# WHU-USI3DV/LaneMapping

Hardware: AMD Instinct MI355X
Metric: BEV tiles/sec end-to-end (LAS points -> polylines) (higher is better)
Workload: dtype f32; 1 GPU; on-GPU LAS->BEV raster (4,194,304 points/tile resident in HBM) + configs/Proj_polyline_fpn_vit_vertex_2.py, batch=16 per GPU, seeded random weights; lines_per_tile=45, streams=2, hip_graphs=True, points=resident, stream_check=not run (--full runs it), gather_check=n/a (1 rank), raster_check=not run (--full runs it), dist_ranks=1, rccl_ranks=1

## Files before the change

### lanemapping_amd/csrc/vit.hip

```cpp
#include "common.h"

namespace {

constexpr int DH = 64;
constexpr int QC = 36;
constexpr int KLD = DH + 1;
constexpr size_t VALU_STATIC_LDS = 272;
constexpr size_t LDS_PER_WG = 160 * 1024;
constexpr size_t valu_dynamic_lds(int N) { return ((size_t)N * KLD + (size_t)QC * (N + 4) + QC * DH) * sizeof(float); }
constexpr bool valu_fits(int N) { return valu_dynamic_lds(N) + VALU_STATIC_LDS <= LDS_PER_WG; }
static_assert(valu_fits(380) && !valu_fits(381), "the VALU kernel holds 380 keys (163312 + 272 B), not 381 (163716 + 272 B > 163840)");
static_assert(valu_fits(64), "the masked entry's 64 tokens fit");

__global__ __launch_bounds__(256) void attention_kernel(const float* __restrict__ qkv, float* __restrict__ out, int NT,
                                                        int heads, float scale, const int* __restrict__ valid) {
    extern __shared__ __attribute__((aligned(16))) float smem[];
    __shared__ int kidx[64];
    __shared__ int kcount;
    const int tid = threadIdx.x;
    const int q0 = blockIdx.x * QC, h = blockIdx.y, b = blockIdx.z;
    const int inner = heads * DH;
    const long row0 = (long)b * NT;
    const int ld = 3 * inner;
    int N = NT;
    if (valid) {
        if (tid < 64) {
            const bool v = tid < NT && valid[(long)b * NT + tid] != 0;
            const unsigned long long m = __ballot(v);
            if (v) kidx[__popcll(m & ((1ull << tid) - 1ull))] = tid;
            if (tid == 0) kcount = (int)__popcll(m);
        }
        __syncthreads();
        N = kcount;
        if (N == 0) {
            for (int i = tid; i < QC * DH; i += 256) {
                const int n = q0 + (i >> 6);
                if (n < NT) out[(row0 + n) * inner + h * DH + (i & 63)] = 0.f;
            }
            return;
        }
    }
    const int SLD = N + 4;
    float* KV = smem;
    float* S = KV + N * KLD;
    float* Q = S + QC * SLD;
#define LM_KROW(n) (valid ? kidx[n] : (n))

    for (int i = tid; i < N * DH; i += 256) {
        const int n = i >> 6, d = i & 63;
        KV[n * KLD + d] = qkv[(row0 + LM_KROW(n)) * ld + inner + h * DH + d];
    }
    for (int i = tid; i < QC * DH; i += 256) {
        const int n = i >> 6, d = i & 63;
        Q[i] = (q0 + n < NT) ? qkv[(row0 + q0 + n) * ld + h * DH + d] : 0.f;
    }
    __syncthreads();
    for (int idx = tid; idx < QC * N; idx += 256) {
        const int i = idx / N, j = idx - i * N;
        const float* qr = Q + i * DH;
        const float* kr = KV + j * KLD;
        float acc = 0.f;
#pragma unroll
        for (int d = 0; d < DH; ++d) acc = fmaf(qr[d], kr[d], acc);
        S[i * SLD + j] = acc * scale;
    }
    __syncthreads();
    for (int i = tid; i < N * DH; i += 256) {
        const int n = i >> 6, d = i & 63;
        KV[n * KLD + d] = qkv[(row0 + LM_KROW(n)) * ld + 2 * inner + h * DH + d];
    }
#undef LM_KROW
    const int wave = tid >> 6, lane = tid & 63;
    for (int i = wave; i < QC; i += 4) {
        float* sr = S + i * SLD;
        float m = -INFINITY;
        for (int j = lane; j < N; j += 64) m = fmaxf(m, sr[j]);
        for (int o = 32; o > 0; o >>= 1) m = fmaxf(m, __shfl_xor(m, o));
        float sum = 0.f;
        for (int j = lane; j < N; j += 64) {
            const float e = expf(sr[j] - m);
            sr[j] = e;
            sum += e;
        }
        for (int o = 32; o > 0; o >>= 1) sum += __shfl_xor(sum, o);
        const float inv = 1.0f / sum;
        for (int j = lane; j < N; j += 64) sr[j] *= inv;
    }
    __syncthreads();
    const int d = lane;
    float acc[QC / 4];
#pragma unroll
    for (int r = 0; r < QC / 4; ++r) acc[r] = 0.f;
    for (int j = 0; j < N; ++j) {
        const float v = KV[j * KLD + d];
#pragma unroll
        for (int r = 0; r < QC / 4; ++r) acc[r] = fmaf(S[(wave + 4 * r) * SLD + j], v, acc[r]);
    }
#pragma unroll
    for (int r = 0; r < QC / 4; ++r) {
        const int i = q0 + wave + 4 * r;
        if (i < NT) out[(row0 + i) * inner + h * DH + d] = acc[r];
    }
}

typedef float f32x16 __attribute__((ext_vector_type(16)));
typedef float f32x4 __attribute__((ext_vector_type(4)));
constexpr int NKB = 11;
constexpr int NPAD = NKB * 32;
constexpr int KP = DH + 4;

__global__ __launch_bounds__(256) void attention_mfma_kernel(const float* __restrict__ qkv, float* __restrict__ out, int N, int heads,
                                                             float scale) {
    extern __shared__ __attribute__((aligned(16))) float smem[];
    const int tid = threadIdx.x, lane = tid & 63, wave = tid >> 6;
    const int h = blockIdx.y, b = blockIdx.z;
    const int inner = heads * DH, ld = 3 * inner;
    const long row0 = (long)b * N;
    const int col = lane & 31, half = lane >> 5;
    const int q = (blockIdx.x * 4 + wave) * 32 + col;
    for (int i = tid; i < NPAD * (DH / 4); i += 256) {
        const int n = i >> 4, c4 = (i & 15) * 4;
        f32x4 v = {0.f, 0.f, 0.f, 0.f};
        if (n < N) v = *reinterpret_cast<const f32x4*>(qkv + (row0 + n) * ld + inner + h * DH + c4);
        *reinterpret_cast<f32x4*>(smem + n * KP + c4) = v;
    }
    f32x4 qf[8];
#pragma unroll
    for (int g = 0; g < 8; ++g) {
        qf[g] = f32x4{0.f, 0.f, 0.f, 0.f};
        if (q < N) qf[g] = *reinterpret_cast<const f32x4*>(qkv + (row0 + q) * ld + h * DH + 8 * g + 4 * half);
    }
    __syncthreads();
    f32x16 s[NKB];
#pragma unroll
    for (int kb = 0; kb < NKB; ++kb) {
#pragma unroll
        for (int r = 0; r < 16; ++r) s[kb][r] = 0.f;
#pragma unroll
        for (int g = 0; g < 8; ++g) {
            const f32x4 kf = *reinterpret_cast<const f32x4*>(smem + (kb * 32 + col) * KP + 8 * g + 4 * half);
#pragma unroll
            for (int t = 0; t < 4; ++t) s[kb] = __builtin_amdgcn_mfma_f32_32x32x2f32(kf[t], qf[g][t], s[kb], 0, 0, 0);
        }
    }
    float m = -INFINITY;
#pragma unroll
    for (int kb = 0; kb < NKB; ++kb)
#pragma unroll
        for (int r = 0; r < 16; ++r) {
            const int key = kb * 32 + (r & 3) + 8 * (r >> 2) + 4 * half;
            s[kb][r] = key < N ? s[kb][r] * scale : -INFINITY;
            m = fmaxf(m, s[kb][r]);
        }
    m = fmaxf(m, __shfl_xor(m, 32));
    float sum = 0.f;
#pragma unroll
    for (int kb = 0; kb < NKB; ++kb)
#pragma unroll
        for (int r = 0; r < 16; ++r) {
            const float e = expf(s[kb][r] - m);
            s[kb][r] = e;
            sum += e;
        }
    sum += __shfl_xor(sum, 32);
    __syncthreads();
    for (int i = tid; i < NPAD * (DH / 4); i += 256) {
        const int n = i >> 4, c4 = (i & 15) * 4;
        f32x4 v = {0.f, 0.f, 0.f, 0.f};
        if (n < N) v = *reinterpret_cast<const f32x4*>(qkv + (row0 + n) * ld + 2 * inner + h * DH + c4);
        *reinterpret_cast<f32x4*>(smem + n * DH + c4) = v;
    }
    __syncthreads();
    f32x16 o[2];
#pragma unroll
    for (int dt = 0; dt < 2; ++dt)
#pragma unroll
        for (int r = 0; r < 16; ++r) o[dt][r] = 0.f;
#pragma unroll
    for (int kb = 0; kb < NKB; ++kb)
#pragma unroll
        for (int r = 0; r < 16; ++r) {
            const float* vrow = smem + (kb * 32 + (r & 3) + 8 * (r >> 2) + 4 * half) * DH + col;
            o[0] = __builtin_amdgcn_mfma_f32_32x32x2f32(vrow[0], s[kb][r], o[0], 0, 0, 0);
            o[1] = __builtin_amdgcn_mfma_f32_32x32x2f32(vrow[32], s[kb][r], o[1], 0, 0, 0);
        }
    if (q < N) {
        const float inv = 1.0f / sum;
        float* orow = out + (row0 + q) * inner + h * DH;
#pragma unroll
        for (int dt = 0; dt < 2; ++dt)
#pragma unroll
            for (int r4 = 0; r4 < 4; ++r4) {
                f32x4 v = {o[dt][4 * r4] * inv, o[dt][4 * r4 + 1] * inv, o[dt][4 * r4 + 2] * inv, o[dt][4 * r4 + 3] * inv};
                *reinterpret_cast<f32x4*>(orow + dt * 32 + 8 * r4 + 4 * half) = v;
            }
    }
}

constexpr int FKB = 64;
constexpr int VP = DH + 8;

__global__ __launch_bounds__(256) __attribute__((amdgpu_waves_per_eu(4))) void attention_flash_kernel(
    const float* __restrict__ qkv, float* __restrict__ out, int N, int heads, float scale) {
    extern __shared__ __attribute__((aligned(16))) float smem[];
    float* Ks = smem;
    float* Vs = smem + FKB * KP;
    const int tid = threadIdx.x, lane = tid & 63, wave = tid >> 6;
    const int h = blockIdx.y, b = blockIdx.z;
    const int inner = heads * DH, ld = 3 * inner;
    const long row0 = (long)b * N;
    const int col = lane & 31, half = lane >> 5;
    const int q = (blockIdx.x * 4 + wave) * 32 + col;
    f32x4 qf[8];
#pragma unroll
    for (int g = 0; g < 8; ++g) {
        qf[g] = f32x4{0.f, 0.f, 0.f, 0.f};
        if (q < N) qf[g] = *reinterpret_cast<const f32x4*>(qkv + (row0 + q) * ld + h * DH + 8 * g + 4 * half);
    }
    f32x16 o[2];
#pragma unroll
    for (int dt = 0; dt < 2; ++dt)
#pragma unroll
        for (int r = 0; r < 16; ++r) o[dt][r] = 0.f;
    float m = -INFINITY, l = 0.f;
    for (int k0 = 0; k0 < N; k0 += FKB) {
        __syncthreads();
        for (int i = tid; i < FKB * (DH / 4); i += 256) {
            const int n = i >> 4, c4 = (i & 15) * 4;
            f32x4 kv = {0.f, 0.f, 0.f, 0.f}, vv = {0.f, 0.f, 0.f, 0.f};
            if (k0 + n < N) {
                const float* src = qkv + (row0 + k0 + n) * ld + inner + h * DH + c4;
                kv = *reinterpret_cast<const f32x4*>(src);
                vv = *reinterpret_cast<const f32x4*>(src + inner);
            }
            *reinterpret_cast<f32x4*>(Ks + n * KP + c4) = kv;
            *reinterpret_cast<f32x4*>(Vs + n * VP + c4) = vv;
        }
        __syncthreads();
#pragma unroll
        for (int sb = 0; sb < FKB / 32; ++sb) {
            const int kb0 = k0 + sb * 32;
            if (kb0 >= N) break;
            f32x16 s;
#pragma unroll
            for (int r = 0; r < 16; ++r) s[r] = 0.f;
#pragma unroll
            for (int g = 0; g < 8; ++g) {
                const f32x4 kf = *reinterpret_cast<const f32x4*>(Ks + (sb * 32 + col) * KP + 8 * g + 4 * half);
#pragma unroll
                for (int t = 0; t < 4; ++t) s = __builtin_amdgcn_mfma_f32_32x32x2f32(kf[t], qf[g][t], s, 0, 0, 0);
            }
            float mb = m;
#pragma unroll
            for (int r = 0; r < 16; ++r) {
                const int key = kb0 + (r & 3) + 8 * (r >> 2) + 4 * half;
                s[r] = key < N ? s[r] * scale : -INFINITY;
                mb = fmaxf(mb, s[r]);
            }
            mb = fmaxf(mb, __shfl_xor(mb, 32));
            const float alpha = expf(m - mb);
            m = mb;
            float ps = 0.f;
#pragma unroll
            for (int r = 0; r < 16; ++r) {
                s[r] = expf(s[r] - m);
                ps += s[r];
            }
            l = l * alpha + ps;
            o[0] *= alpha;
            o[1] *= alpha;
#pragma unroll
            for (int r = 0; r < 16; ++r) {
                const float* vrow = Vs + (sb * 32 + (r & 3) + 8 * (r >> 2) + 4 * half) * VP + col;
                o[0] = __builtin_amdgcn_mfma_f32_32x32x2f32(vrow[0], s[r], o[0], 0, 0, 0);
                o[1] = __builtin_amdgcn_mfma_f32_32x32x2f32(vrow[32], s[r], o[1], 0, 0, 0);
            }
        }
    }
    l += __shfl_xor(l, 32);
    if (q < N) {
        const float inv = 1.0f / l;
        float* orow = out + (row0 + q) * inner + h * DH;
#pragma unroll
        for (int dt = 0; dt < 2; ++dt)
#pragma unroll
            for (int r4 = 0; r4 < 4; ++r4) {
                f32x4 v = {o[dt][4 * r4] * inv, o[dt][4 * r4 + 1] * inv, o[dt][4 * r4 + 2] * inv, o[dt][4 * r4 + 3] * inv};
                *reinterpret_cast<f32x4*>(orow + dt * 32 + 8 * r4 + 4 * half) = v;
            }
    }
}

}

LM_API int lm_attention_f32(void* stream, const float* qkv, float* out, int B, int N, int heads, int dim_head, float scale) {
    LM_REQUIRE(qkv && out, "attention: null pointer");
    LM_REQUIRE(dim_head == DH, "attention: dim_head=%d must be %d", dim_head, DH);
    if (N > NPAD - 32 && N <= NPAD) {
        const size_t lds_m = (size_t)NPAD * KP * sizeof(float);
        if (int e = lm_ensure_dynamic_lds((const void*)attention_mfma_kernel, lds_m)) return e;
        hipLaunchKernelGGL(attention_mfma_kernel, dim3(lm_cdiv(lm_cdiv(N, 32), 4), heads, B), dim3(256), lds_m, (hipStream_t)stream, qkv, out,
                           N, heads, scale);
        LM_LAUNCH_CHECK();
        return LM_OK;
    }
    LM_REQUIRE(N >= 1, "attention: N=%d must be at least 1", N);
    if (!valu_fits(N)) {
        const size_t lds_f = (size_t)FKB * (KP + VP) * sizeof(float);
        if (int e = lm_ensure_dynamic_lds((const void*)attention_flash_kernel, lds_f)) return e;
        hipLaunchKernelGGL(attention_flash_kernel, dim3(lm_cdiv(lm_cdiv(N, 32), 4), heads, B), dim3(256), lds_f, (hipStream_t)stream, qkv,
                           out, N, heads, scale);
        LM_LAUNCH_CHECK();
        return LM_OK;
    }
    const size_t lds = valu_dynamic_lds(N);
    if (int e = lm_ensure_dynamic_lds((const void*)attention_kernel, lds)) return e;
    hipLaunchKernelGGL(attention_kernel, dim3(lm_cdiv(N, QC), heads, B), dim3(256), lds, (hipStream_t)stream, qkv, out, N, heads, scale,
                       (const int*)nullptr);
    LM_LAUNCH_CHECK();
    return LM_OK;
}

LM_API int lm_attention_masked_f32(void* stream, const float* qkv, float* out, const int* valid, int B, int N, int heads, int dim_head,
                                   float scale) {
    LM_REQUIRE(qkv && out && valid, "attention_masked: null pointer");
    LM_REQUIRE(dim_head == DH && N >= 1 && N <= 64, "attention_masked: dim_head=%d must be %d, N=%d at most 64", dim_head, DH, N);
    const size_t lds = valu_dynamic_lds(N);
    if (int e = lm_ensure_dynamic_lds((const void*)attention_kernel, lds)) return e;
    hipLaunchKernelGGL(attention_kernel, dim3(lm_cdiv(N, QC), heads, B), dim3(256), lds, (hipStream_t)stream, qkv, out, N, heads, scale, valid);
    LM_LAUNCH_CHECK();
    return LM_OK;
}
```

Before: 401.4 tiles/s.

## Stage MFMA attention keys/values in two halves to halve LDS footprint

Adds a default attention path for the padded 352-key case that stages K, then V, into LDS in two chunks (6 then 5 key blocks) instead of holding the whole head's keys at once. This shrinks dynamic LDS per workgroup so two workgroups can co-reside, and the kernel is tagged with waves_per_eu 2. It adds extra barriers and reloads, and the whole-head path stays reachable through an environment variable. Register pressure from keeping all 11 score tiles live may limit the occupancy gain.

Result: no change. 398.9 tiles/s, median of 2 (-0.6%).

```diff
diff --git a/lanemapping_amd/csrc/vit.hip b/lanemapping_amd/csrc/vit.hip
--- a/lanemapping_amd/csrc/vit.hip
+++ b/lanemapping_amd/csrc/vit.hip
@@ -1,4 +1,6 @@
 #include "common.h"
+
+#include <cstdlib>
 
 namespace {
 
@@ -109,9 +111,8 @@
 constexpr int NPAD = NKB * 32;
 constexpr int KP = DH + 4;
 
-__global__ __launch_bounds__(256) void attention_mfma_kernel(const float* __restrict__ qkv, float* __restrict__ out, int N, int heads,
-                                                             float scale) {
-    extern __shared__ __attribute__((aligned(16))) float smem[];
+__device__ __forceinline__ void attention_mfma_whole_head(float* smem , const float* __restrict__ qkv,
+                                                          float* __restrict__ out, int N, int heads, float scale) {
     const int tid = threadIdx.x, lane = tid & 63, wave = tid >> 6;
     const int h = blockIdx.y, b = blockIdx.z;
     const int inner = heads * DH, ld = 3 * inner;
@@ -195,6 +196,139 @@
                 *reinterpret_cast<f32x4*>(orow + dt * 32 + 8 * r4 + 4 * half) = v;
             }
     }
+}
+
+constexpr int NKB0 = 6;
+static_assert(NKB0 * 2 >= NKB, "the second half fits the buffer of the first");
+constexpr int TAIL0 = 2 * (NKB - 1 - NKB0);
+
+template <int NKBS, int BATCH, int GUARD>
+__device__ __forceinline__ void attn_stage(float* smem, const float* __restrict__ src, int ld, int nvalid, int pitch, int tid) {
+    constexpr int PASSES = NKBS * 2;
+    static_assert(PASSES % BATCH == 0, "whole batches");
+    const int n0 = tid >> 4, c4 = (tid & 15) * 4;
+    const unsigned voff = (unsigned)(n0 * ld + c4);
+#pragma unroll
+    for (int i0 = 0; i0 < PASSES; i0 += BATCH) {
+        f32x4 v[BATCH];
+#pragma unroll
+        for (int j = 0; j < BATCH; ++j) {
+            const float* rows = src + (long)(16 * (i0 + j)) * ld;
+            v[j] = f32x4{0.f, 0.f, 0.f, 0.f};
+            if (i0 + j < GUARD || n0 + 16 * (i0 + j) < nvalid) v[j] = *reinterpret_cast<const f32x4*>(rows + voff);
+        }
+#pragma unroll
+        for (int j = 0; j < BATCH; ++j) *reinterpret_cast<f32x4*>(smem + (n0 + 16 * (i0 + j)) * pitch + c4) = v[j];
+    }
+}
+
+__device__ __forceinline__ void attention_mfma_halves(float* smem ,
+                                                      const float* __restrict__ qkv, float* __restrict__ out, int N, int heads, float scale) {
+    const int tid = threadIdx.x, lane = tid & 63;
+    const int wave = __builtin_amdgcn_readfirstlane(tid >> 6);
+    const int h = blockIdx.y, b = blockIdx.z;
+    const int inner = heads * DH, ld = 3 * inner;
+    const long row0 = (long)b * N;
+    const int col = lane & 31, half = lane >> 5;
+    const int q = (blockIdx.x * 4 + wave) * 32 + col;
+    const bool live = (blockIdx.x * 4 + wave) * 32 < N;
+    const float* const kv = qkv + row0 * ld + inner + h * DH;
+    attn_stage<NKB0, 2 * NKB0, 2 * NKB0>(smem, kv, ld, N, KP, tid);
+    f32x4 qf[8];
+#pragma unroll
+    for (int g = 0; g < 8; ++g) {
+        qf[g] = f32x4{0.f, 0.f, 0.f, 0.f};
+        if (q < N) qf[g] = *reinterpret_cast<const f32x4*>(qkv + (row0 + q) * ld + h * DH + 8 * g + 4 * half);
+    }
+    __syncthreads();
+    f32x16 s[NKB];
+#pragma unroll
+    for (int part = 0; part < 2; ++part) {
+        if (part == 1) {
+            __syncthreads();
+            attn_stage<NKB - NKB0, 2 * (NKB - NKB0), TAIL0>(smem, kv + (long)NKB0 * 32 * ld, ld, N - NKB0 * 32, KP, tid);
+            __syncthreads();
+        }
+        if (live) {
+#pragma unroll
+            for (int kb = part ? NKB0 : 0; kb < (part ? NKB : NKB0); ++kb) {
+                const int lb = part ? kb - NKB0 : kb;
+#pragma unroll
+                for (int r = 0; r < 16; ++r) s[kb][r] = 0.f;
+#pragma unroll
+                for (int g = 0; g < 8; ++g) {
+                    const f32x4 kf = *reinterpret_cast<const f32x4*>(smem + (lb * 32 + col) * KP + 8 * g + 4 * half);
+#pragma unroll
+                    for (int t = 0; t < 4; ++t) s[kb] = __builtin_amdgcn_mfma_f32_32x32x2f32(kf[t], qf[g][t], s[kb], 0, 0, 0);
+                }
+            }
+        }
+    }
+    float sum = 0.f;
+    if (live) {
+        float m = -INFINITY;
+#pragma unroll
+        for (int kb = 0; kb < NKB; ++kb)
+#pragma unroll
+            for (int r = 0; r < 16; ++r) {
+                const int key = kb * 32 + (r & 3) + 8 * (r >> 2) + 4 * half;
+                s[kb][r] = key < N ? s[kb][r] * scale : -INFINITY;
+                m = fmaxf(m, s[kb][r]);
+            }
+        m = fmaxf(m, __shfl_xor(m, 32));
+#pragma unroll
+        for (int kb = 0; kb < NKB; ++kb)
+#pragma unroll
+            for (int r = 0; r < 16; ++r) {
+                const float e = expf(s[kb][r] - m);
+                s[kb][r] = e;
+                sum += e;
+            }
+        sum += __shfl_xor(sum, 32);
+    }
+    f32x16 o[2];
+#pragma unroll
+    for (int dt = 0; dt < 2; ++dt)
+#pragma unroll
+        for (int r = 0; r < 16; ++r) o[dt][r] = 0.f;
+#pragma unroll
+    for (int part = 0; part < 2; ++part) {
+        __syncthreads();
+        if (part == 0) attn_stage<NKB0, NKB0, 2 * NKB0>(smem, kv + inner, ld, N, DH, tid);
+        else attn_stage<NKB - NKB0, NKB - NKB0, TAIL0>(smem, kv + inner + (long)NKB0 * 32 * ld, ld, N - NKB0 * 32, DH, tid);
+        __syncthreads();
+        if (live) {
+#pragma unroll
+            for (int kb = part ? NKB0 : 0; kb < (part ? NKB : NKB0); ++kb) {
+                const int lb = part ? kb - NKB0 : kb;
+#pragma unroll
+                for (int r = 0; r < 16; ++r) {
+                    const float* vrow = smem + (lb * 32 + (r & 3) + 8 * (r >> 2) + 4 * half) * DH + col;
+                    o[0] = __builtin_amdgcn_mfma_f32_32x32x2f32(vrow[0], s[kb][r], o[0], 0, 0, 0);
+                    o[1] = __builtin_amdgcn_mfma_f32_32x32x2f32(vrow[32], s[kb][r], o[1], 0, 0, 0);
+                }
+            }
+        }
+    }
+    if (q < N) {
+        const float inv = 1.0f / sum;
+        float* orow = out + (row0 + q) * inner + h * DH;
+#pragma unroll
+        for (int dt = 0; dt < 2; ++dt)
+#pragma unroll
+            for (int r4 = 0; r4 < 4; ++r4) {
+                f32x4 v = {o[dt][4 * r4] * inv, o[dt][4 * r4 + 1] * inv, o[dt][4 * r4 + 2] * inv, o[dt][4 * r4 + 3] * inv};
+                *reinterpret_cast<f32x4*>(orow + dt * 32 + 8 * r4 + 4 * half) = v;
+            }
+    }
+}
+
+template <bool HALVES>
+__global__ __launch_bounds__(256) __attribute__((amdgpu_waves_per_eu(HALVES ? 2 : 1))) void attention_mfma_kernel(
+    const float* __restrict__ qkv, float* __restrict__ out, int N, int heads, float scale) {
+    extern __shared__ __attribute__((aligned(16))) float smem[];
+    if (HALVES) attention_mfma_halves(smem, qkv, out, N, heads, scale);
+    else attention_mfma_whole_head(smem, qkv, out, N, heads, scale);
 }
 
 constexpr int FKB = 64;
@@ -297,9 +431,18 @@
     LM_REQUIRE(qkv && out, "attention: null pointer");
     LM_REQUIRE(dim_head == DH, "attention: dim_head=%d must be %d", dim_head, DH);
     if (N > NPAD - 32 && N <= NPAD) {
+        static const bool whole_head = [] { const char* e = getenv("LM_ATTN_WHOLE_HEAD"); return e && atoi(e) != 0; }();
+        if (!whole_head) {
+            const size_t lds_h = (size_t)NKB0 * 32 * KP * sizeof(float);
+            if (int e = lm_ensure_dynamic_lds((const void*)attention_mfma_kernel<true>, lds_h)) return e;
+            hipLaunchKernelGGL(attention_mfma_kernel<true>, dim3(lm_cdiv(lm_cdiv(N, 32), 4), heads, B), dim3(256), lds_h, (hipStream_t)stream,
+                               qkv, out, N, heads, scale);
+            LM_LAUNCH_CHECK();
+            return LM_OK;
+        }
         const size_t lds_m = (size_t)NPAD * KP * sizeof(float);
-        if (int e = lm_ensure_dynamic_lds((const void*)attention_mfma_kernel, lds_m)) return e;
-        hipLaunchKernelGGL(attention_mfma_kernel, dim3(lm_cdiv(lm_cdiv(N, 32), 4), heads, B), dim3(256), lds_m, (hipStream_t)stream, qkv, out,
+        if (int e = lm_ensure_dynamic_lds((const void*)attention_mfma_kernel<false>, lds_m)) return e;
+        hipLaunchKernelGGL(attention_mfma_kernel<false>, dim3(lm_cdiv(lm_cdiv(N, 32), 4), heads, B), dim3(256), lds_m, (hipStream_t)stream, qkv, out,
                            N, heads, scale);
         LM_LAUNCH_CHECK();
         return LM_OK;
```
